# cornellius-gp/linear_operator

Hardware: AMD Instinct MI355X
Metric: cg_member_matvecs_per_sec (higher is better)
Workload: dtype f32

## Files before the change

linear_operator_amd/csrc/lo_cg.hip:

```cpp
#include <algorithm>
#include <chrono>
#include <cstddef>
#include <cmath>
#include <atomic>
#include <cstdlib>
#include <cstring>
#include <new>

#include "lo_device.h"
#include "lo_internal.h"
#include "lo_cg_onchip.h"

namespace lo {

bool g_onchip_disabled = false;
int g_onchip_fused_timeouts = 0;
constexpr int kResidentBackoff0 = 16, kResidentBackoffMax = 4096;
static std::atomic<int> g_res_timeouts{0}, g_res_cooldown{0}, g_res_backoff{kResidentBackoff0}, g_res_rearms{0},
    g_res_inject{0};
bool resident_off() { return g_onchip_disabled || g_res_cooldown.load(std::memory_order_relaxed) > 0; }
void resident_tick() {
  int c = g_res_cooldown.load(std::memory_order_relaxed);
  while (c > 0 && !g_res_cooldown.compare_exchange_weak(c, c - 1, std::memory_order_relaxed)) {
  }
  if (c == 1) {
    g_res_rearms.fetch_add(1, std::memory_order_relaxed);
    fprintf(stderr, "liblo_amd: resident kernels re-armed after their cool-down\n");
  }
}
static void resident_untick() {
  int c = g_res_cooldown.load(std::memory_order_relaxed);
  while (c > 0 && !g_res_cooldown.compare_exchange_weak(c, c + 1, std::memory_order_relaxed)) {
  }
}
static bool resident_off_after_tick() { return g_onchip_disabled || g_res_cooldown.load(std::memory_order_relaxed) > 1; }
static void resident_return_injection() { g_res_inject.fetch_add(1, std::memory_order_relaxed); }
void resident_note_ok() { g_res_backoff.store(kResidentBackoff0, std::memory_order_relaxed); }
bool resident_take_injection() {
  int n = g_res_inject.load(std::memory_order_relaxed);
  while (n > 0 && !g_res_inject.compare_exchange_weak(n, n - 1, std::memory_order_relaxed)) {
// ... 80 lines not shown

constexpr int kLockstepMinCols = 4;

struct CgDev {
  int64_t B, N;
  int c, S, S_dot, S_rz;
  int n_tridiag, max_iter, n_tridiag_iter, T;
  float tol, eps, stop_after;
  int check_nan_first;
  float *x, *r, *p, *z, *Ap;
  float *pAp_part, *rr_part, *rz_part;
  float *rhs_norm, *rz, *alpha, *beta, *resid_norm, *prev_ar, *prev_beta;
  int *rhs_is_zero, *has_conv;
  float* t_mat;
  CgCtrl* ctrl;
  float* ctrl_part;
  unsigned long long* oc_gbuf;
  unsigned long long* oc_close;
  unsigned long long* ls_gbuf;
  unsigned long long* pf_gbuf;
  int* pf_ctr;
  unsigned long long* pf_gran;
  unsigned long long* sc_gbuf;
  int* sc_ctr;
  unsigned long long* sc_gran;
  int* oc_err;
  float* oc_resid;
  int* oc_init_conv;
  float* oc_zero_q;
  float* oc_ones;
  float* oc_ab;
  int* oc_maxoff;
  long long* oc_dbg;
  double* rs_ws;
};

__global__ __launch_bounds__(kThreads) void k_cg_init_scal(CgDev d, const float* __restrict__ part) {
  const int64_t n = d.B * d.c;
  for (int64_t i = threadIdx.x; i < n; i += kThreads) {
    const int64_t b = i / d.c;
    const int col = (int)(i % d.c);
    float acc = 0.f;
    for (int s = 0; s < d.S; ++s) acc += part[(b * d.S + s) * d.c + col];
    float nrm = sqrtf(acc);
    const int zero = nrm < d.eps;
    d.rhs_is_zero[i] = zero;
    d.rhs_norm[i] = zero ? 1.0f : nrm;
  }
}

__global__ __launch_bounds__(kThreads) void k_cg_init_vec(CgDev d, const float* __restrict__ rhs,
                                                           const float* __restrict__ x0, int rows_per) {
  const int s = blockIdx.x, b = blockIdx.y;
  const int c = d.c, N = (int)d.N;
  const int nrs = kThreads / c;
  const int col = threadIdx.x % c, slot = threadIdx.x / c;
  if (slot >= nrs) return;
  const int r0 = s * rows_per, r1 = min(N, r0 + rows_per);
  const float nrm = d.rhs_norm[(size_t)b * c + col];
  const size_t base = (size_t)b * N * c + col;
  for (int row = r0 + slot; row < r1; row += nrs) {
    const size_t i = base + (size_t)row * c;
    d.r[i] = rhs[i] / nrm;
    d.x[i] = x0 ? x0[i] / nrm : 0.f;
  }
}
// ... 375 lines not shown
      cg_step_cols_worthwhile(B, N, c, pre != nullptr))
    out->streaming_precond = pre ? LO_STREAM_PRE_FUSED_COLS : LO_STREAM_NOPRE_FUSED_COLS;
  const bool opaque = (op->kind == LO_OP_CALLBACK) || pre_cb;
  out->poll_chunk = (opaque || global_rule) ? 1 : 4;
  const bool root_serial = serial.engine == LO_ENGINE_RESIDENT_ROOT;
  out->needs_q = (pre && !pre->Q && !(oc_ok && (ls_cols == c || root_serial))) ? 1 : 0;
  if (!oc_ok) return;
  out->resident = 1;
  out->resident_iterations = kfloor0 + 1;
  out->lockstep_cols = ls_cols;
  out->lockstep_group = ls_cols ? lockstep_group_size(N) : 0;
  if (ls_cols < c) {
    out->serial_engine = serial.engine;
    out->serial_group = serial.group;
  }
  out->lean = (!global_rule && !sw.keep_state && (ls_cols == c || root_serial)) ? 1 : 0;
  const bool rs_base = pre && pre->RS && pre_root && pre->rf_ld == RC && !global_rule && !sw.keep_state;
  if (rs_base && sh.rs_cols && (c >= 2 || prm->n_tridiag > 0) && !sw.no_rspace_cols) {
    out->rspace = 1;
    out->lean = 1;
  } else if (rs_base && out->lean && ls_cols == 0 && c == 1 && prm->n_tridiag == 0 && pre->E && root_serial &&
             rspace_eligible(RC, N, c) && !sw.no_rspace && !sw.no_wrec) {
    out->rspace = 2;
  }
}


static int oc_record_iters(const lo_cg_params* prm) {
  const int fmi0 = prm->floor_max_iter > 0 ? prm->floor_max_iter : prm->max_iter;
  int oc_iters = std::min(10, fmi0 - 1);
  if (prm->n_tridiag) oc_iters = std::max(oc_iters, std::min(prm->max_tridiag_iter, fmi0 - 1));
  return std::max(1, oc_iters + 1);
}

constexpr size_t kCgTail = 1024;
static int cg_layout(Arena& ar, const lo_op_desc* op, const lo_precond_desc* pre, bool pre_cb, const lo_cg_params* prm,
                     CgDev* d, MatvecPlan* pl, lo_matvec_cb mv_cb, void* mv_user, PrecondPlan* pp, hipStream_t st) {
  const int64_t B = op->B, N = op->N, c = prm->c;
  Split sp = choose_split(B, N, 256);
  const size_t nv = (size_t)B * N * c;
  const bool precond = pre != nullptr || pre_cb;
  CgDev& dd = *d;
  dd.B = B; dd.N = N; dd.c = (int)c; dd.S = sp.S;
  dd.ctrl = ar.take<CgCtrl>(1);
  dd.oc_gbuf = ar.take<unsigned long long>(std::max(onchip_gbuf_bytes(66), rspace_gbuf_bytes(std::max(66 * 8, 2 * onchip_num_workgroups()))) / sizeof(unsigned long long));
  dd.oc_close = ar.take<unsigned long long>((size_t)B + 2);
  dd.x = ar.take<float>(nv);
  dd.r = ar.take<float>(nv);
  dd.p = ar.take<float>(nv);
  dd.Ap = ar.take<float>(nv);
  dd.z = precond ? ar.take<float>(nv) : nullptr;
  dd.S_dot = matvec_S_dot(op, c, sp);
  dd.pAp_part = ar.take<float>((size_t)B * std::max(dd.S_dot, sp.S) * c);
  dd.rr_part = ar.take<float>((size_t)B * sp.S * c);
  dd.rz_part = precond ? ar.take<float>((size_t)B * sp.S * c) : dd.rr_part;
  dd.S_rz = sp.S;
  const size_t ns = (size_t)B * c;
  dd.rhs_norm = ar.take<float>(ns);
  dd.rz = ar.take<float>(ns);
  dd.alpha = ar.take<float>(ns);
  dd.beta = ar.take<float>(ns);
  dd.resid_norm = ar.take<float>(ns);
  dd.rhs_is_zero = ar.take<int>(ns);
  dd.has_conv = ar.take<int>(ns);
  const size_t nt = (size_t)B * std::max(1, (int)prm->n_tridiag);
  dd.prev_ar = ar.take<float>(nt);
  dd.prev_beta = ar.take<float>(nt);
  dd.ctrl_part = ar.take<float>(3 * 256);
  dd.oc_err = dd.ctrl ? &dd.ctrl->oc_err : nullptr;
  const int oc_iters = oc_record_iters(prm);
  const CgShape shp = cg_shape(op, pre, pre_cb, prm);
  const bool oc_shape = shp.oc_shape;
  const size_t oc_n = oc_shape ? (size_t)B * c : 1;
  dd.oc_resid = ar.take<float>(oc_n * oc_iters);
  dd.oc_init_conv = ar.take<int>(oc_n);
  dd.oc_ab = shp.has_ab ? ar.take<float>(2 * oc_n * oc_iters) : nullptr;
  dd.oc_maxoff = ar.take<int>((size_t)std::max(1, (int)prm->max_tridiag_iter) + 1);
  dd.oc_dbg = ar.take<long long>(16);
  dd.rs_ws = shp.rs_cols ? ar.take<double>(rspace_cols_ws_doubles(B, N, padded_rank(op->R), (int)c)) : nullptr;
  dd.ls_gbuf = shp.has_ls_gbuf
                   ? ar.take<unsigned long long>(lockstep_gbuf_bytes(32, 16) / sizeof(unsigned long long))
                   : nullptr;
  const bool pf_shape = shp.pf_shape;
  dd.pf_gbuf = pf_shape ? ar.take<unsigned long long>(precond_fused_gbuf_bytes() / sizeof(unsigned long long)) : nullptr;
  dd.pf_ctr = pf_shape ? ar.take<int>(2 * ((size_t)std::max(1, (int)prm->max_iter) + 1)) : nullptr;
  dd.pf_gran = pf_shape ? ar.take<unsigned long long>((size_t)B) : nullptr;
  dd.sc_gbuf = shp.sc_alloc ? ar.take<unsigned long long>(cg_step_cols_gbuf_bytes() / sizeof(unsigned long long)) : nullptr;
  dd.sc_ctr = shp.sc_alloc ? ar.take<int>(2 * ((size_t)std::max(1, (int)prm->max_iter) + 1)) : nullptr;
  dd.sc_gran = shp.sc_alloc ? ar.take<unsigned long long>(3 * (size_t)B) : nullptr;
  dd.oc_zero_q = nullptr;
  dd.oc_ones = nullptr;
  if (shp.has_zero_q) {
    dd.oc_zero_q = ar.take<float>((size_t)B * N * 4);
    dd.oc_ones = ar.take<float>((size_t)B);
  }
  int rc = pre ? precond_plan_init(pp, pre, B, N, c, sp, &ar, st) : LO_OK;
  const int rc_mv = matvec_plan_init(pl, op, mv_cb, mv_user, c, sp, &ar, st);
  if (!rc) rc = rc_mv;
  if (!rc && pl->S_dot != dd.S_dot) rc = LO_ERR_LAUNCH;
  return (rc || ar.ok) ? rc : LO_ERR_WORKSPACE;
}

struct CgDebug {
  bool ls = false, oc = false, sc = false;
  int member = 0;
  static CgDebug read(const CgEnv& env, int64_t B) {
    const bool ls = env.ls_debug && B >= 8, oc = !ls && env.oc_debug && B >= 8;
    return {ls, oc, env.sc_debug, oc ? env.oc_member : (ls ? env.ls_member : 0)};
  }
  int report_resident(const long long* dev) const {
    long long ts[12];
    if (ls) {
      LO_HIP_CHECK(hipMemcpy(ts, dev, 10 * sizeof(long long), hipMemcpyDeviceToHost));
      fprintf(stderr, "lockstep item (100 MHz ticks): load+H %lld init %lld iters %lld store %lld | direction %lld "
              "alpha+x+r %lld reduce-mfma %lld cross-wave %lld group-sum %lld\n",
              ts[1] - ts[0], ts[2] - ts[1], ts[3] - ts[2], ts[4] - ts[3], ts[5], ts[6], ts[7], ts[8], ts[9]);
    }
    if (oc) {
      LO_HIP_CHECK(hipMemcpy(ts, dev, 12 * sizeof(long long), hipMemcpyDeviceToHost));
      if (ts[8] || ts[9])
        fprintf(stderr, "  root-form kernel phases: updates %lld, w partials + all-reduce %lld, first-wave algebra %lld\n",
                ts[8], ts[9], ts[10]);
      fprintf(stderr, "onchip member0 (100 MHz ticks): load %lld init %lld iters %lld store %lld | wg-wait %lld publish %lld poll %lld\n",
              ts[1] - ts[0], ts[2] - ts[1], ts[3] - ts[2], ts[4] - ts[3], ts[5], ts[6], ts[7]);
    }
    return LO_OK;
  }
  int report_streaming(const long long* dev) const {
    if (!sc) return LO_OK;
    long long ts[8];
    LO_HIP_CHECK(hipMemcpy(ts, dev, sizeof(ts), hipMemcpyDeviceToHost));
    if (ts[5])
      fprintf(stderr, "cg_step_cols member 0, first workgroup (100 MHz ticks per launch): loads+alpha %.1f update+mfma %.1f "
              "all-reduce %.1f beta+control %.1f p %.1f\n", (double)ts[0] / ts[5], (double)ts[1] / ts[5], (double)ts[2] / ts[5],
              (double)ts[3] / ts[5], (double)ts[4] / ts[5]);
    return LO_OK;
  }
};

struct CgSolve {
  const lo_op_desc* op;
  const lo_precond_desc* pre;
  lo_matvec_cb precond_cb;
  void* precond_user;
  const lo_cg_params* prm;
  const float *rhs, *x0;
  float* x;
  hipStream_t st;
  int64_t B, N;
  int c;
  CgDev d;
  MatvecPlan pl;
  PrecondPlan pp = {};
  Split sp;
  int fmi, oc_nwg;
  bool precond, global_rule, oc_nopre;
  CgSwitches sw;
// ... 93 lines not shown
};

static int resident_close(CgSolve& s, const OnchipArgs& a, bool lean, bool dense, bool rs_cols_ran, unsigned close_ticket,
                          OcNext* next) {
  CgDev& d = s.d; const lo_cg_params* prm = s.prm; hipStream_t st = s.st; CgCtrl& h = s.h;
  const int ktri = prm->n_tridiag ? std::min(a.iters, (int)prm->max_tridiag_iter) : 0;
  const unsigned tri_grid = (unsigned)(((size_t)s.B * std::max(1, (int)prm->n_tridiag) + kThreads - 1) / kThreads);
  if (ktri) {
    LO_HIP_CHECK(hipMemsetAsync(d.oc_maxoff, 0, sizeof(int) * (prm->max_tridiag_iter + 1), st));
    hipLaunchKernelGGL(k_oc_maxoff, dim3(tri_grid), s.block, 0, st, d, d.oc_ab, ktri);
  }
  CgCtrl* mirror = static_cast<CgCtrl*>(pinned_status_block());
  const unsigned ticket = close_ticket ? close_ticket : next_ticket();
  if (!close_ticket)
    hipLaunchKernelGGL(k_cg_ctrl_onchip, dim3(1), s.block, 0, st, d, d.oc_resid, d.oc_init_conv, a.iters, ktri, mirror,
                       ticket);
  if (ktri) hipLaunchKernelGGL(k_oc_tridiag, dim3(tri_grid), s.block, 0, st, d, d.oc_ab, ktri);
  LO_LAUNCH_CHECK();
  if (mirror) {
    if (ktri) LO_HIP_CHECK(hipStreamSynchronize(st));
    else if (wait_ticket(reinterpret_cast<volatile unsigned*>(mirror) + 63, ticket, st)) return LO_ERR_LAUNCH;
    if (g_prof_host) tls_host_ticket = std::chrono::steady_clock::now();
    memcpy(&h, mirror, sizeof(CgCtrl));
  } else {
    LO_HIP_CHECK(hipMemcpyAsync(&h, d.ctrl, sizeof(CgCtrl), hipMemcpyDeviceToHost, st));
    LO_HIP_CHECK(hipStreamSynchronize(st));
  }
  int rc = LO_OK;
  if (h.oc_err == 0) {
    if (s.owned_launch) handoff_launch_confirm(s.owned_launch);
    rc = cg_global_check(s);
    if (rc) return rc;
  }
  rc = s.dbg.report_resident(d.oc_dbg);
  if (rc) return rc;
  if (h.oc_err == 0 && lean && h.rs_redo && tls_rspace_diag_ran && !dense) {
    *next = OcNext::kRedoDense;
  } else if (h.oc_err == 0 && lean && !h.stop) {
    lean_miss_note(s.op, prm, s.pre ? s.pre->generation : 0);
    if (s.pre && !s.pre->Q) return LO_ERR_UNSUPPORTED;
    *next = OcNext::kRedoState;
  } else if (h.oc_err == 0) {
    s.k_start = a.iters; s.x_written = true;
    resident_note_ok();
    lo_cg_plan& ex = s.exec;
    ex.resident = 1;
    if (rs_cols_ran) ex.lockstep_cols = 0, ex.serial_engine = LO_ENGINE_NONE;
    ex.lean = lean ? 1 : 0;
    ex.rspace = rs_cols_ran ? 1 : ((lean && tls_rspace_resident_ran) ? 2 : 0);
    ex.rspace_diag = (ex.rspace == 2 && tls_rspace_diag_ran) ? 1 : 0;
    *next = OcNext::kDone;
  } else {
    fprintf(stderr, "liblo_amd: operator-resident CG timed out, falling back to the streaming engine\n");
    onchip_note_timeout();
    if (s.ws_cleared) LO_HIP_CHECK(hipMemsetAsync(d.ctrl, 0, sizeof(CgCtrl), st));
    memset(&h, 0, sizeof(h));
    *next = OcNext::kStream;
  }
  return LO_OK;
}

static int resident_attempt(CgSolve& s, int attempt, bool lean, bool dense, OcNext* next) {
  CgDev& d = s.d; const lo_precond_desc* pre = s.pre; const lo_cg_params* prm = s.prm; lo_cg_plan& ex = s.exec;
  const int64_t B = s.B, N = s.N; const int c = s.c, RC = s.pl.lr.R4, ocR4 = s.oc_nopre ? 4 : s.pp.R4;
  hipStream_t st = s.st;
  *next = OcNext::kStream;
  OnchipArgs a;
  a.C = s.pl.lr.Apad; a.d = s.op->d; a.d_mode = s.op->diag_mode;
  if (s.oc_nopre) {
    if (ex.lockstep_cols < c && ex.serial_engine == LO_ENGINE_RESIDENT_GEN2) {
      LO_HIP_CHECK(hipMemsetAsync(d.oc_zero_q, 0, sizeof(float) * (size_t)B * N * 4, st));
      LO_HIP_CHECK(hipMemsetD32Async((hipDeviceptr_t)d.oc_ones, 0x3f800000, (size_t)B, st));
    }
    a.Q = d.oc_zero_q; a.dinv = d.oc_ones; a.dinv_mode = LO_DIAG_CONST;
  } else {
    a.Q = s.pp.Qp; a.dinv = pre->dinv; a.dinv_mode = pre->constant_diag ? LO_DIAG_CONST : LO_DIAG_FULL;
  }
  a.rhs = s.rhs; a.B = B; a.N = (int)N; a.c = c; a.ab_rec = prm->n_tridiag ? d.oc_ab : nullptr;
  a.col0 = 0; a.ncols = c; a.RK = s.pp.R4; a.RCg = RC;
  a.F = nullptr; a.EF = nullptr; a.E = nullptr; a.RS = nullptr; a.RSD = nullptr;
  a.close_gran = nullptr; a.close_count = nullptr; a.close_ctrl = nullptr; a.close_mirror = nullptr;
  a.close_ticket = 0; a.close_tol = 0.f; a.close_floor_ok = 0;
  a.close_epoch = 0x80000000u; a.tag_base = 0; a.handoff_owned = 0;
  a.iters = s.plan.first_stop_iteration + 1; a.eps = prm->eps; a.stop_after = prm->stop_updating_after;
  a.x = d.x; a.r = d.r; a.p = d.p; a.z = d.z;
  auto lean_state = [&](bool on) {
    a.x = on ? nullptr : d.x; a.r = on ? nullptr : d.r; a.p = on ? nullptr : d.p; a.z = on ? nullptr : d.z;
  };
  a.rhs_norm = d.rhs_norm; a.rz = d.rz; a.alpha = d.alpha; a.beta = d.beta; a.resid_norm = d.resid_norm;
  a.rhs_is_zero = d.rhs_is_zero; a.has_conv = d.has_conv;
  a.resid_rec = d.oc_resid; a.init_conv = d.oc_init_conv; a.err = d.oc_err;
  a.allow_l2_handoff = onchip_l2_handoff_allowed();
  a.prefetch = 1;
  a.dbg = nullptr; a.dbg_member = s.dbg.member;
  const bool injected = attempt == 0 && resident_take_injection();
  const bool inject = s.sw.oc_test_fallback || injected;
  s.owned_launch = 0;
  if (inject && s.ws_cleared) LO_HIP_CHECK(hipMemsetAsync(d.oc_err, 1, 1, st));
  if (s.dbg.oc || s.dbg.ls) LO_HIP_CHECK(hipMemsetAsync(d.oc_dbg, 0, 16 * sizeof(long long), st));
  int rc = LO_OK; int ls = ex.lockstep_cols;
  bool rs_cols_ran = false;
  unsigned close_ticket = 0;
  if (s.plan.rspace == 1 && lean && d.rs_ws) {
    a.xout = s.x;
    lean_state(true);
    a.F = pre->F; a.EF = pre->EF; a.E = pre->E; a.RS = pre->RS; a.RSD = pre->RSD;
    rc = rspace_cols_launch(RC, a, d.rs_ws, st);
    if (rc == LO_OK) {
      rs_cols_ran = true;
      ls = 0;
    } else if (rc != LO_ERR_UNSUPPORTED) {
      return rc;
    }
  }
  if (ls) {
    a.ncols = ls;
    a.xout = s.x;
    lean_state(lean);
    a.gbuf = d.ls_gbuf; a.next_member = d.oc_err + 2;
    a.dbg = s.dbg.ls ? d.oc_dbg : nullptr;
    LO_HIP_CHECK(hipMemsetAsync(d.ls_gbuf, 0, lockstep_gbuf_bytes(32, 16), st));
    a.GW = ex.lockstep_group;
    a.RW = (int)((N + a.GW - 1) / a.GW);
    rc = lockstep_launch(RC, pre != nullptr, a, std::min(s.oc_nwg, 256), st);
    if (rc == LO_ERR_UNSUPPORTED && a.GW == 16) {
      a.GW = ex.lockstep_group = 8;
      a.RW = (int)((N + 7) / 8);
      rc = lockstep_launch(RC, pre != nullptr, a, std::min(s.oc_nwg, 256), st);
    }
    if (rc == LO_ERR_UNSUPPORTED) {
      ex.lockstep_cols = ls = 0;
      ex.lockstep_group = 0;
// ... 595 lines not shown
```

linear_operator_amd/csrc/lo_cg_onchip.h:

```cpp
#pragma once
#include <stdint.h>

#include <hip/hip_runtime.h>

namespace lo {

struct CgCtrl;

struct OnchipArgs {
  const float* C;
  const float* Q;
  const float* d;
  const float* dinv;
  int d_mode, dinv_mode;
  const float* rhs;
  int c;
  int col0, ncols;
  int RK;
  int RCg;
  const float* F;
  const float* EF;
  const float* E;
  const double* RS;
  const double* RSD;
  float* ab_rec;
  int64_t B;
  int N, RW;
  int GW;
  int iters;
  float eps, stop_after;
  float *x, *r, *p, *z;
  float* xout;
  float *rhs_norm, *rz, *alpha, *beta, *resid_norm;
  int *rhs_is_zero, *has_conv;
  float* resid_rec;
  int* init_conv;
  unsigned long long* gbuf;
  int* err;
  int* next_member;
  int prefetch;
  int allow_l2_handoff;
  unsigned long long* close_gran;
  int* close_count;
  unsigned close_epoch;
  unsigned tag_base;
  int handoff_owned;
  struct CgCtrl* close_ctrl;
  struct CgCtrl* close_mirror;
  unsigned close_ticket;
  float close_tol;
  int close_floor_ok;
  long long* dbg;
  int dbg_member;
};

int onchip4_launch(int RC, int RK, const OnchipArgs& a, int nwg, hipStream_t st);
int onchip5_launch(int RC, const OnchipArgs& a, int nwg, hipStream_t st);
bool onchip5_eligible(int RC, int64_t N, int64_t c);
int rspace_launch(int RC, const OnchipArgs& a, int nwg, hipStream_t st);
int rspace3_launch(int RC, const OnchipArgs& a, int nwg, hipStream_t st);
int rspace3_launch_owned(int RC, const OnchipArgs& a, int nwg, bool inject, unsigned* launch_id, hipStream_t st);
void handoff_launch_confirm(unsigned launch_id);
bool rspace_eligible(int RC, int64_t N, int64_t c);
size_t rspace_gbuf_bytes(int nworkgroups);
extern thread_local bool tls_rspace_diag_ran;
extern thread_local bool tls_rspace_resident_ran;
int rspace_cols_launch(int RC, const OnchipArgs& a, double* ws, hipStream_t st);
bool rspace_cols_eligible(int RC, int64_t N, int64_t c);
size_t rspace_cols_ws_doubles(int64_t B, int64_t N, int RC, int c);
int lockstep_launch(int RC, bool pre, const OnchipArgs& a, int nwg, hipStream_t st);
bool lockstep_eligible(int RC, int RK, bool pre, int64_t N, int64_t ncols);
size_t lockstep_gbuf_bytes(int ngroups, int GW);
int lockstep_group_size(int64_t N);

}
```

linear_operator_amd/csrc/lo_rspace3.hip:

```cpp
#include <algorithm>
#include <atomic>
#include <mutex>
#include <type_traits>
#include <stdlib.h>

#include "lo_device.h"
#include "lo_internal.h"
#include "lo_cg_onchip.h"
#include "lo_group_reduce.h"
#include "lo_cg_close.h"
#include "lo_f64_lanes.h"

namespace lo {

namespace {

typedef float f32x4 __attribute__((ext_vector_type(4)));
typedef __attribute__((address_space(1))) const f32x4 g_cf4;
typedef __attribute__((address_space(1))) const float g_cf;
typedef __attribute__((address_space(1))) float g_f;
typedef __attribute__((address_space(1))) const char g_cc;
template <class T>
__device__ __forceinline__ T* opaque_uniform(T* p) {
  asm volatile("" : "+s"(p));
// ... 9 lines not shown
  long long member_off;
};
PeerOut g_peer_out = {{nullptr, nullptr, nullptr, nullptr, nullptr, nullptr, nullptr}, 0, 0};
std::mutex g_peer_mu;

__host__ __device__ constexpr int r3_np(int RC) { return 2 * RC + 6; }

__device__ __forceinline__ unsigned xor4_dpp_u(unsigned x) {
  const int a = __builtin_amdgcn_update_dpp(0, (int)x, 0x104, 0xf, 0x5, false);
  return (unsigned)__builtin_amdgcn_update_dpp(a, (int)x, 0x114, 0xf, 0xa, false);
}
__device__ __forceinline__ double halve4_d(double lo, double hi, int lane) {
  const bool up = (lane & 4) != 0;
  const double keep = up ? hi : lo;
  const double send = up ? lo : hi;
  return keep + mk_d(xor4_dpp_u(lo_w(send)), xor4_dpp_u(hi_w(send)));
}

template <int CH>
__device__ __forceinline__ double rows_reduce_d(double (&p)[CH], int lane) {
  if constexpr (CH == 8) {
#pragma unroll
    for (int m = 0; m < 4; ++m) p[m] = halve4_d(p[m], p[m + 4], lane);
    p[0] = halve_pair_d<2>(p[0], p[2], lane);
    p[1] = halve_pair_d<2>(p[1], p[3], lane);
    return halve_pair_d<1>(p[0], p[1], lane);
  } else if constexpr (CH == 4) {
    p[0] = halve_pair_d<2>(p[0], p[2], lane);
    p[1] = halve_pair_d<2>(p[1], p[3], lane);
    return halve_pair_d<1>(p[0], p[1], lane);
  } else {
    return halve_pair_d<1>(p[0], p[1], lane);
  }
}

template <int RC, int GW>
__global__ __launch_bounds__(R3_TPB, 2) void k_cg_rspace3(OnchipArgs a, PeerOut po) {
  constexpr int CH = RC / 4;
  constexpr int RPI = 64 / CH;
  constexpr int NI = 256 / RPI;
  constexpr int NP = r3_np(RC);
  constexpr int MLD = RC + 2;
  constexpr int NH = RC / 2;
  constexpr int NG = 2 * GW * NP;
  __shared__ __attribute__((aligned(16))) float bst[4][256];
  __shared__ __attribute__((aligned(16))) float dst[4][256];
  __shared__ __attribute__((aligned(16))) double mat_s[3 * RC * MLD];
  __shared__ __attribute__((aligned(16))) double red[4][NP];
  __shared__ __attribute__((aligned(16))) double res[NP];
  __shared__ __attribute__((aligned(16))) double gv[4][32];
  __shared__ unsigned polw[GW > 1 ? NG : 2];
  const GroupPlace gp = group_place(GW, (int)gridDim.x / 8);
  if (!gp.active) return;
  const int grp = gp.grp, wig = gp.wig, ngroups = gp.ngroups;
  const int t = threadIdx.x, lane = t & 63, wave = t >> 6;
  const int wave_u = __builtin_amdgcn_readfirstlane(wave);
  unsigned long long* const gbase = a.gbuf + (size_t)grp * 2 * NG;
  unsigned tag = a.tag_base;
  bool same_xcd = false;
  const unsigned xcc = xcc_id();
  bool first = true;
  const int row0 = wig * R3_ROWS + 256 * wave_u;
  const int row0c = max(0, min(row0, a.N - 256));
  const bool di_full = a.dinv_mode == LO_DIAG_FULL;
  float* const bw = bst[wave_u];
  float* const dw = dst[wave_u];
  constexpr int NPF = 8;
  f32x4 pre[NPF];
  constexpr int NXT = NI - NPF;
  f32x4 nxt[NXT > 0 ? NXT : 1];
  auto request = [&](int64_t bm, int tl_, int i_lo, auto cnt, f32x4* dst) {
    const int ln_ = tl_ & 63, k_ = ln_ & (CH - 1), g_ = ln_ / CH;
    const unsigned loff = (unsigned)((g_ * RC + 4 * k_) * sizeof(float));
    g_cc* Cw = (g_cc*)(a.C + ((size_t)bm * a.N + row0c) * RC);
#pragma unroll
    for (int q = 0; q < decltype(cnt)::value / 8; ++q) {
      g_cc* bq = opaque_uniform(Cw + (i_lo + 8 * q + 4) * 1024);
#pragma unroll
      for (int i = 0; i < 8; ++i) dst[8 * q + i] = *(g_cf4*)(bq + loff + (i - 4) * 1024);
    }
  };
  int64_t b = grp;
  {
    int tl0 = t;
    asm volatile("" : "+v"(tl0));
    if (b < a.B) {
      request(b, tl0, 0, std::integral_constant<int, NPF>{}, pre);
      request(b, tl0, NPF, std::integral_constant<int, NXT>{}, nxt);
    } else {
#pragma unroll
      for (int i = 0; i < NPF; ++i) pre[i] = (f32x4){0.f, 0.f, 0.f, 0.f};
    }
  }
  while (b < a.B) {
    const bool stamp = a.dbg && b == a.dbg_member && wig == 0 && t == 0;
    if (stamp) a.dbg[0] = wall_clock64();
    int drawn = 0;
    if (wig == 0 && t == 0) drawn = atomicAdd(a.next_member, 1);
    int tl = t;
    asm volatile("" : "+v"(tl));
    const int ln = tl & 63, k = ln & (CH - 1), g = ln / CH;
    f32x4 Cr[NI];
#pragma unroll
    for (int i = 0; i < NPF; ++i) Cr[i] = pre[i];
#pragma unroll
    for (int i = 0; i < NXT; ++i) Cr[NPF + i] = nxt[i];
    float bq4[4], dq4[4];
    {
      g_cf* bb_ = opaque_uniform((g_cf*)(a.rhs + (size_t)b * a.N + row0c));
      g_cf* dd_ = opaque_uniform((g_cf*)(di_full ? a.dinv + (size_t)b * a.N + row0c : a.dinv + b));
      const int lo_e = row0 - row0c, hi_e = max(0, min(256, a.N - row0c));
      const int dstride = di_full ? 1 : 0;
#pragma unroll
      for (int m = 0; m < 4; ++m) {
        const int e = ln + 64 * m;
        const bool own = e >= lo_e && e < hi_e;
        bq4[m] = own ? bb_[e] : 0.f;
        dq4[m] = own ? dd_[e * dstride] : 0.f;
      }
    }
    constexpr int NM = (3 * RC * RC / 2 + R3_TPB - 1) / R3_TPB;
    f32x4 mv[NM];
    {
      typedef __attribute__((address_space(1))) const f32x4 g_m4;
      const g_m4* src = (const g_m4*)(a.RSD + (size_t)b * 6 * RC * RC);
#pragma unroll
      for (int u = 0; u < NM; ++u) {
        const int e = min(tl + R3_TPB * u, 3 * RC * RC / 2 - 1);
        const int ms = e / (RC * RC / 2);
        const int mg = ms == 0 ? 0 : ms + 1;
        mv[u] = src[(size_t)mg * (RC * RC / 2) + (e - ms * (RC * RC / 2))];
      }
    }
    const double lam_mine = a.RSD[((size_t)b * 6 + 5) * RC * RC + min(ln & 31, RC - 1)];
#pragma unroll
    for (int m = 0; m < 4; ++m) {
      bw[ln + 64 * m] = bq4[m];
      dw[ln + 64 * m] = dq4[m];
    }
#pragma unroll
    for (int u = 0; u < NM; ++u) {
      const int e = tl + R3_TPB * u;
      if (e < 3 * RC * RC / 2) {
        const int mi = e / (RC / 2), jj = e % (RC / 2);
        *reinterpret_cast<f32x4*>(&mat_s[mi * MLD + 2 * jj]) = mv[u];
      }
    }
    __builtin_amdgcn_wave_barrier();
    if (stamp) a.dbg[1] = wall_clock64();

    {
      double aw[4] = {0.0, 0.0, 0.0, 0.0}, au[4] = {0.0, 0.0, 0.0, 0.0};
#pragma unroll
      for (int i0 = 0; i0 < NI; i0 += 4) {
#pragma unroll
        for (int i = i0; i < i0 + 4; ++i) {
          const int r = RPI * i + g;
          const double bb = (double)bw[r];
          const double bd = bb * (double)dw[r];
          const double c0 = (double)Cr[i].x, c1 = (double)Cr[i].y, c2 = (double)Cr[i].z, c3 = (double)Cr[i].w;
          aw[0] = fma(c0, bd, aw[0]); au[0] = fma(c0, bb, au[0]);
          aw[1] = fma(c1, bd, aw[1]); au[1] = fma(c1, bb, au[1]);
          aw[2] = fma(c2, bd, aw[2]); au[2] = fma(c2, bb, au[2]);
          aw[3] = fma(c3, bd, aw[3]); au[3] = fma(c3, bb, au[3]);
        }
        __builtin_amdgcn_sched_barrier(0);
      }
      double s_acc = 0.0, a_acc = 0.0, d2_acc = 0.0;
#pragma unroll
      for (int j = 0; j < 4; ++j) {
        const int rw = 64 * j + RPI * k + g;
        const double bb = (double)bw[rw], di = (double)dw[rw];
        s_acc = fma(bb, bb * di, s_acc);
        a_acc = fma(bb, bb, a_acc);
        d2_acc = fma(di, di, d2_acc);
      }
      double h0 = halve_pair_d<32>(aw[0], au[0], ln), h1 = halve_pair_d<32>(aw[1], au[1], ln);
      double h2 = halve_pair_d<32>(aw[2], au[2], ln), h3 = halve_pair_d<32>(aw[3], au[3], ln);
      h0 = halve_pair_d<16>(h0, h2, ln);
      h1 = halve_pair_d<16>(h1, h3, ln);
      double mine = halve_pair_d<8>(h0, h1, ln);
      if constexpr (CH <= 4) mine = bfly_add_d<4>(mine);
// ... 47 lines not shown
              x[q] = granule_load(slot + min(idx, NG - 1));
              ok = ok && (granule_tag(x[q]) == tag);
            }
            if (ok) break;
            if (poll_give_up(spin, a.err)) {
              lost = true;
              break;
            }
            __builtin_amdgcn_s_sleep(1);
          }
#pragma unroll
          for (int q = 0; q < CKQ; ++q) {
            const int idx = tt + R3_TPB * (q0 + q);
            if (idx < NG) polw[idx] = granule_bits(x[q]);
          }
        }
        __syncthreads();
        if (tt < NP) {
          double tot = 0.0;
#pragma unroll
          for (int w = 0; w < GW; ++w) tot += mk_d(polw[(w * NP + tt) * 2], polw[(w * NP + tt) * 2 + 1]);
          res[tt] = tot;
        }
      }
      __syncthreads();
    }
    if (GW > 1 && first) {
      unsigned xc = xcc;
      asm volatile("" : "+s"(xc));
      same_xcd = same_xcd_verdict(res[2 * RC + 4], res[2 * RC + 5], GW, xc, a.allow_l2_handoff);
    }
    first = false;
    if (stamp) a.dbg[2] = wall_clock64();
    const int64_t b_next = (int64_t)res[2 * RC + 2];
    {
      int tp = t;
      asm volatile("" : "+v"(tp));
      if (b_next < a.B) {
        request(b_next, tp, 0, std::integral_constant<int, NPF>{}, pre);
      } else {
#pragma unroll
        for (int i = 0; i < NPF; ++i) pre[i] = (f32x4){0.f, 0.f, 0.f, 0.f};
      }
    }
    if (a.prefetch & 1) __builtin_amdgcn_s_setprio(3);

    const int j = lane & 31, hf = lane >> 5;
    const bool live = j < RC;
    const int jr = live ? j : RC - 1;
    double yj = 0.0, xi = 0.0;
    float nrm;
    {
      double a0 = res[2 * RC + 1], s = res[2 * RC];
      const double d2 = res[2 * RC + 3];
      nrm = sqrtf((float)a0);
      const bool rhs_zero = nrm < a.eps;
      if (rhs_zero) nrm = 1.0f;
      const double inv = 1.0 / (double)nrm;
      const double w0 = live ? res[jr] * inv : 0.0, u0 = live ? res[RC + jr] * inv : 0.0;
      s *= inv * inv;
      a0 *= inv * inv;
      float sa = a.stop_after;
      asm volatile("" : "+s"(sa));
      const double sure_rz = 2.0 * (double)sa * (double)sa * sqrt(d2);
      auto own_row_dot = [&](const double* mrow, const double* vec) {
        double a0_ = 0.0, a1_ = 0.0;
#pragma unroll
        for (int q = 0; q < NH; q += 2) {
          const double2 xa = *reinterpret_cast<const double2*>(mrow + q);
          const double2 xx = *reinterpret_cast<const double2*>(vec + q);
          a0_ = fma(xa.x, xx.x, a0_);
          a1_ = fma(xa.y, xx.y, a1_);
        }
        double lo_, up_;
        halves_d(a0_ + a1_, lo_, up_);
        return lo_ + up_;
      };
      double* myv = gv[wave];
      if (hf == 0) myv[j] = w0;
      __builtin_amdgcn_wave_barrier();
      const double* row0m = mat_s + (size_t)jr * MLD + hf * NH;
      double c0 = own_row_dot(row0m, myv + hf * NH);
      double e0 = own_row_dot(row0m + (size_t)1 * RC * MLD, myv + hf * NH);
      const double* nrow = row0m + (size_t)2 * RC * MLD;
      const double* tucol = mat_s + (size_t)(1 * RC + hf * NH) * MLD + jr;
      c0 = live ? c0 : 0.0;
      e0 = live ? e0 : 0.0;
      double tau2 = s - lanes32_sum_d(c0 * e0);
      tau2 = tau2 > 0.0 ? tau2 : 0.0;
      const bool delicate = !rhs_zero && tau2 < 1e-2 * s;
      const double lam = live ? lam_mine : 1.0;
      long long ts_a = 0, ts_b = 0;
      if (stamp) ts_a = wall_clock64();
      double cj = c0, qj = 0.0, etaj = 0.0;
      double cp = 1.0, qp = 0.0, etap = 0.0;
      double rz = 0.0, pApE = 0.0, alpha = 0.0, beta = 0.0;
      float rn = 0.f, last_alpha = 0.f;
      bool conv = false;
      unsigned close_flags = 0u;
      const size_t bc = (size_t)b;
      const bool rec = wig == 0 && lane == 0;
      const int last_owner = (a.iters - 1) & 3;
      for (int kk = -1; kk < a.iters; ++kk) {
        if (kk >= 0) {
          last_alpha = (float)alpha;
          etaj = fma(alpha, qj, etaj);
          etap = fma(alpha, qp, etap);
          cj = fma(-alpha * lam, qj, cj);
          cp = fma(-alpha, qp, cp);
        }
        const double lc = lam * cj;
        const bool lo_h = hf == 0;
        const float inv_rz = __builtin_amdgcn_rcpf((float)rz);
        const double red2 = row16_sum_d(halve_pair_d<16>(lo_h ? cj * cj : lc * qj, lo_h ? lc * cj : 0.0, lane));
        const auto pick = [&](double v, int ln_) {
          return mk_d((unsigned)__builtin_amdgcn_readlane((int)lo_w(v), ln_),
                      (unsigned)__builtin_amdgcn_readlane((int)hi_w(v), ln_));
        };
        const double cc = pick(red2, 0), clc = pick(red2, 16), clq = pick(red2, 32);
        const double rzn = fma(cp * cp, tau2, cc);
        const bool sure = rzn > sure_rz;
        const bool rec_first = kk == 0 && a.close_gran == nullptr && wave == 0;
        const bool rec_last = kk == a.iters - 1 && wave == last_owner;
        const bool own = rec_first || rec_last || !sure;
        float rnn = 0.f;
        if (kk < 0) {
          const float s1f = (float)a0;
          rnn = __builtin_amdgcn_sqrtf(s1f < 0.f ? 0.f : s1f);
        } else if (own) {
          const double dl = fma(-cp, c0, cj);
          __builtin_amdgcn_wave_barrier();
          if (hf == 0) myv[j] = dl;
          __builtin_amdgcn_wave_barrier();
          double gj_;
          {
            double a0_ = 0.0, a1_ = 0.0;
#pragma unroll
            for (int q = 0; q < NH; q += 2) {
              const double2 dd = *reinterpret_cast<const double2*>(myv + hf * NH + q);
              a0_ = fma(tucol[(size_t)q * MLD], dd.x, a0_);
              a1_ = fma(tucol[(size_t)(q + 1) * MLD], dd.y, a1_);
            }
            double lo_, up_;
            halves_d(a0_ + a1_, lo_, up_);
            gj_ = live ? lo_ + up_ : 0.0;
          }
          __builtin_amdgcn_wave_barrier();
          if (hf == 0) myv[j] = gj_;
          __builtin_amdgcn_wave_barrier();
          const double nd = own_row_dot(nrow, myv + hf * NH);
          const double r2 = row16_sum_d(halve_pair_d<16>(gj_ * nd, gj_ * u0, lane));
          const double dnd = pick(r2, 0), dm = pick(r2, 16);
          const double s1 = fma(cp, fma(cp, a0, 2.0 * dm), dnd);
          const float s1f = (float)s1;
          rnn = __builtin_amdgcn_sqrtf(s1f < 0.f ? 0.f : s1f);
        }
        if (kk >= 0) {
          beta = ((float)rz < a.eps) ? 0.0 : (double)((float)rzn * inv_rz);
          if (rhs_zero) rnn = 0.f;
          rn = rnn;
          if (rec && (rec_first || rec_last)) a.resid_rec[(size_t)kk * a.B + bc] = rn;
        } else {
          beta = 0.0;
          rn = rnn;
          if (wig == 0 && t == 0) a.init_conv[bc] = (rn < a.stop_after) ? 1 : 0;
          close_flags = ((rn < a.stop_after) ? 1u : 0u) | (delicate ? 4u : 0u);
          if (delicate && rec && wave == 0) atomicOr(a.err + 4, 1);
        }
        if (kk == 0 && (rnn != rnn || rzn != rzn)) close_flags |= 2u;
        conv = (own || rhs_zero) ? (rn < a.stop_after) : false;
        rz = rzn;
        pApE = fma(beta, fma(beta, pApE, 2.0 * clq), clc);
        qj = fma(beta, qj, cj);
        qp = fma(beta, qp, cp);
        const double pAp = fma(qp * qp, tau2, pApE);
        alpha = ((float)pAp < a.eps) ? 0.0 : (double)((float)rz * __builtin_amdgcn_rcpf((float)pAp));
        if (conv) alpha = 0.0;
      }
      if (stamp) ts_b = wall_clock64();
      if (rec && wave == last_owner) {
        a.rhs_norm[bc] = nrm;
        a.rhs_is_zero[bc] = rhs_zero ? 1 : 0;
        a.rz[bc] = (float)rz;
        a.alpha[bc] = last_alpha;
        a.beta[bc] = (float)beta;
        a.resid_norm[bc] = rn;
        a.has_conv[bc] = conv ? 1 : 0;
        if (a.close_gran) {
          granule_store(a.close_gran + b, granule_pack(a.close_epoch | close_flags, rn), false);
        }
      }
      __builtin_amdgcn_wave_barrier();
      if (hf == 0) myv[j] = fma(-etap, e0, etaj);
      __builtin_amdgcn_wave_barrier();
      xi = etap;
      {
        const double* col = mat_s + (size_t)(hf * NH) * MLD + jr;
        double a0_ = 0.0, a1_ = 0.0;
#pragma unroll
        for (int q = 0; q < NH; q += 2) {
          const double2 ee = *reinterpret_cast<const double2*>(myv + hf * NH + q);
          a0_ = fma(col[(size_t)q * MLD], ee.x, a0_);
          a1_ = fma(col[(size_t)(q + 1) * MLD], ee.y, a1_);
        }
        double lo_, up_;
        halves_d(a0_ + a1_, lo_, up_);
        yj = lo_ + up_;
      }
      yj = live ? yj : 0.0;
      if (stamp) {
        a.dbg[5] = ts_a - a.dbg[2];
        a.dbg[6] = ts_b - ts_a;
        a.dbg[7] = wall_clock64() - ts_b;
      }
      __builtin_amdgcn_wave_barrier();
      if (hf == 0) myv[j] = yj * (double)nrm;
      __builtin_amdgcn_wave_barrier();
    }
    if (!(a.prefetch & 2)) __builtin_amdgcn_s_setprio(0);
    if (stamp) a.dbg[3] = wall_clock64();
    {
      int l2 = lane;
      asm volatile("" : "+v"(l2));
      const int k2 = l2 & (CH - 1), g2 = l2 / CH;
      const double* myv = gv[wave];
      const double2 ya = *reinterpret_cast<const double2*>(&myv[4 * k2]);
      const double2 yb = *reinterpret_cast<const double2*>(&myv[4 * k2 + 2]);
      g_f* const xb = opaque_uniform((g_f*)(a.xout + (size_t)b * a.N + row0c));
      const bool more = b_next < a.B;
      g_cc* const Cn = (g_cc*)(a.C + ((size_t)(more ? b_next : b) * a.N + row0c) * RC);
      const unsigned loffn = (unsigned)((g2 * RC + 4 * k2) * sizeof(float));
#pragma unroll
      for (int js = 0; js < 4; ++js) {
        constexpr int J0 = NPF / CH;
        const int jj = (js + J0) & 3;
        double p[CH];
#pragma unroll
        for (int m = 0; m < CH; ++m) {
          const f32x4 c4 = Cr[CH * jj + m];
          p[m] = fma((double)c4.w, yb.y, fma((double)c4.z, yb.x, fma((double)c4.y, ya.y, (double)c4.x * ya.x)));
        }
        const double xv = rows_reduce_d<CH>(p, l2);
        const int rw = 64 * jj + RPI * k2 + g2;
        const int row = row0c + rw;
        const double acc = fma(xi, (double)bw[rw], xv);
        if (row >= row0 && row < a.N) {
          const float xval = (float)(acc * (double)dw[rw]);
          xb[rw] = xval;
          for (int pp = 0; pp < po.n; ++pp)
            ((g_f*)po.buf[pp])[((size_t)(b + po.member_off)) * a.N + row] = xval;
        }
        if (CH * jj >= NPF) {
          g_cc* bqn = opaque_uniform(Cn + (CH * jj + 4) * 1024);
#pragma unroll
          for (int m = 0; m < CH; ++m)
            nxt[CH * jj - NPF + m] = more ? *(g_cf4*)(bqn + loffn + (m - 4) * 1024) : (f32x4){0.f, 0.f, 0.f, 0.f};
        }
      }
      __builtin_amdgcn_wave_barrier();
    }
    __builtin_amdgcn_s_setprio(0);
    if (stamp) a.dbg[4] = wall_clock64();
    __syncthreads();
    b = b_next;
  }
  if (a.close_gran && wig == 0) cg_close_solve(a, ngroups, t);
}

int rspace3_prio() {
  static const int prio = [] {
    const char* e = getenv("LO_RS_PRIO");
    return e ? atoi(e) : 3;
  }();
  return prio;
}

constexpr size_t HO_MAX_WGS = 2 * 320;
constexpr size_t HO_GRAN_PER_WG = 432;
constexpr size_t HO_MAX_MEMBERS = 65536;
constexpr size_t HO_HEAD_BYTES = 256;
constexpr unsigned HO_TAG_LIMIT = 0xfff00000u;
constexpr unsigned HO_EPOCH_LIMIT = 0x1ffffff0u;
struct HandoffBlock {
  char* buf = nullptr;
  size_t bytes = 0;
  bool failed = false;
  unsigned next_tag = 1, next_epoch = 1;
  unsigned last_launch = 0;
  std::atomic<unsigned> confirmed{0};
  bool force_clear = false;
  unsigned clears = 0, launches = 0;
};
HandoffBlock g_handoff[16];
std::atomic<unsigned> g_handoff_ids{0};

HandoffBlock* handoff_block() {
  int dev = 0;
// ... 148 lines not shown
```

Measured before the change: 36.68 million.

## Defer last-iteration residual record to overlap with next member's load

The final CG iteration's residual walk and record stores are peeled out of the per-member loop and run later. For small group widths they run after the next member's data load begins, using a double-buffered shared-memory matrix image; otherwise they run after the x write-back. This takes the serial tail off the critical path between members, at the cost of doubled LDS for the matrix image, extra shared staging state, and a per-member debug timeline buffer.

```diff
diff --git a/linear_operator_amd/csrc/lo_cg.hip b/linear_operator_amd/csrc/lo_cg.hip
--- a/linear_operator_amd/csrc/lo_cg.hip
+++ b/linear_operator_amd/csrc/lo_cg.hip
@@ -6,6 +6,7 @@
 #include <cstdlib>
 #include <cstring>
 #include <new>
+#include <vector>
 
 #include "lo_device.h"
 #include "lo_internal.h"
@@ -152,6 +153,7 @@
   float* oc_ab;
   int* oc_maxoff;
   long long* oc_dbg;
+  int64_t oc_dbg_members;
   double* rs_ws;
 };
 
@@ -593,6 +595,8 @@
   if (prm->n_tridiag) oc_iters = std::max(oc_iters, std::min(prm->max_tridiag_iter, fmi0 - 1));
   return std::max(1, oc_iters + 1);
 }
+
+static size_t oc_dbg_words(int64_t members) { return kOcDbgHead + (size_t)kOcDbgTimeline * (size_t)members; }
 
 constexpr size_t kCgTail = 1024;
 static int cg_layout(Arena& ar, const lo_op_desc* op, const lo_precond_desc* pre, bool pre_cb, const lo_cg_params* prm,
@@ -637,7 +641,8 @@
   dd.oc_init_conv = ar.take<int>(oc_n);
   dd.oc_ab = shp.has_ab ? ar.take<float>(2 * oc_n * oc_iters) : nullptr;
   dd.oc_maxoff = ar.take<int>((size_t)std::max(1, (int)prm->max_tridiag_iter) + 1);
-  dd.oc_dbg = ar.take<long long>(16);
+  dd.oc_dbg_members = (oc_shape && c == 1) ? B : 0;
+  dd.oc_dbg = ar.take<long long>(oc_dbg_words(dd.oc_dbg_members));
   dd.rs_ws = shp.rs_cols ? ar.take<double>(rspace_cols_ws_doubles(B, N, padded_rank(op->R), (int)c)) : nullptr;
   dd.ls_gbuf = shp.has_ls_gbuf
                    ? ar.take<unsigned long long>(lockstep_gbuf_bytes(32, 16) / sizeof(unsigned long long))
@@ -669,7 +674,7 @@
     const bool ls = env.ls_debug && B >= 8, oc = !ls && env.oc_debug && B >= 8;
     return {ls, oc, env.sc_debug, oc ? env.oc_member : (ls ? env.ls_member : 0)};
   }
-  int report_resident(const long long* dev) const {
+  int report_resident(const long long* dev, int64_t members) const {
     long long ts[12];
     if (ls) {
       LO_HIP_CHECK(hipMemcpy(ts, dev, 10 * sizeof(long long), hipMemcpyDeviceToHost));
@@ -684,6 +689,16 @@
                 ts[8], ts[9], ts[10]);
       fprintf(stderr, "onchip member0 (100 MHz ticks): load %lld init %lld iters %lld store %lld | wg-wait %lld publish %lld poll %lld\n",
               ts[1] - ts[0], ts[2] - ts[1], ts[3] - ts[2], ts[4] - ts[3], ts[5], ts[6], ts[7]);
+      if (members > 0) {
+        std::vector<long long> tl((size_t)kOcDbgTimeline * (size_t)members);
+        LO_HIP_CHECK(hipMemcpy(tl.data(), dev + kOcDbgHead, tl.size() * sizeof(long long), hipMemcpyDeviceToHost));
+        for (int64_t m = 0; m < members; ++m) {
+          const long long* w = tl.data() + (size_t)kOcDbgTimeline * (size_t)m;
+          if (w[0])
+            fprintf(stderr, "rs3-timeline member %lld group %lld stamps %lld %lld %lld %lld %lld\n", (long long)m, w[0] - 1, w[1],
+                    w[2], w[3], w[4], w[5]);
+        }
+      }
     }
     return LO_OK;
   }
@@ -843,7 +858,7 @@
     rc = cg_global_check(s);
     if (rc) return rc;
   }
-  rc = s.dbg.report_resident(d.oc_dbg);
+  rc = s.dbg.report_resident(d.oc_dbg, d.oc_dbg_members);
   if (rc) return rc;
   if (h.oc_err == 0 && lean && h.rs_redo && tls_rspace_diag_ran && !dense) {
     *next = OcNext::kRedoDense;
@@ -903,12 +918,12 @@
   a.resid_rec = d.oc_resid; a.init_conv = d.oc_init_conv; a.err = d.oc_err;
   a.allow_l2_handoff = onchip_l2_handoff_allowed();
   a.prefetch = 1;
-  a.dbg = nullptr; a.dbg_member = s.dbg.member;
+  a.dbg = nullptr; a.dbg_member = s.dbg.member; a.dbg_timeline = d.oc_dbg_members;
   const bool injected = attempt == 0 && resident_take_injection();
   const bool inject = s.sw.oc_test_fallback || injected;
   s.owned_launch = 0;
   if (inject && s.ws_cleared) LO_HIP_CHECK(hipMemsetAsync(d.oc_err, 1, 1, st));
-  if (s.dbg.oc || s.dbg.ls) LO_HIP_CHECK(hipMemsetAsync(d.oc_dbg, 0, 16 * sizeof(long long), st));
+  if (s.dbg.oc || s.dbg.ls) LO_HIP_CHECK(hipMemsetAsync(d.oc_dbg, 0, oc_dbg_words(d.oc_dbg_members) * sizeof(long long), st));
   int rc = LO_OK; int ls = ex.lockstep_cols;
   bool rs_cols_ran = false;
   unsigned close_ticket = 0;
diff --git a/linear_operator_amd/csrc/lo_cg_onchip.h b/linear_operator_amd/csrc/lo_cg_onchip.h
--- a/linear_operator_amd/csrc/lo_cg_onchip.h
+++ b/linear_operator_amd/csrc/lo_cg_onchip.h
@@ -52,7 +52,10 @@
   int close_floor_ok;
   long long* dbg;
   int dbg_member;
+  int64_t dbg_timeline;
 };
+constexpr int kOcDbgHead = 16;
+constexpr int kOcDbgTimeline = 6;
 
 int onchip4_launch(int RC, int RK, const OnchipArgs& a, int nwg, hipStream_t st);
 int onchip5_launch(int RC, const OnchipArgs& a, int nwg, hipStream_t st);
diff --git a/linear_operator_amd/csrc/lo_rspace3.hip b/linear_operator_amd/csrc/lo_rspace3.hip
--- a/linear_operator_amd/csrc/lo_rspace3.hip
+++ b/linear_operator_amd/csrc/lo_rspace3.hip
@@ -65,6 +65,69 @@
   } else {
     return halve_pair_d<1>(p[0], p[1], lane);
   }
+}
+
+__device__ __forceinline__ double pick_d(double v, int ln) {
+  return mk_d((unsigned)__builtin_amdgcn_readlane((int)lo_w(v), ln), (unsigned)__builtin_amdgcn_readlane((int)hi_w(v), ln));
+}
+
+template <int NH>
+__device__ __forceinline__ double half_row_dot_d(const double* mrow, const double* vec) {
+  double a0_ = 0.0, a1_ = 0.0;
+#pragma unroll
+  for (int q = 0; q < NH; q += 2) {
+    const double2 xa = *reinterpret_cast<const double2*>(mrow + q);
+    const double2 xx = *reinterpret_cast<const double2*>(vec + q);
+    a0_ = fma(xa.x, xx.x, a0_);
+    a1_ = fma(xa.y, xx.y, a1_);
+  }
+  double lo_, up_;
+  halves_d(a0_ + a1_, lo_, up_);
+  return lo_ + up_;
+}
+
+template <int RC>
+__device__ __forceinline__ float resid_walk_d(double* vec, const double* tucol, const double* nrow, double cj, double cp,
+                                              double c0, double u0, double a0, bool live, int j, int hf, int lane) {
+  constexpr int MLD = RC + 2, NH = RC / 2;
+  const double dl = fma(-cp, c0, cj);
+  __builtin_amdgcn_wave_barrier();
+  if (hf == 0) vec[j] = dl;
+  __builtin_amdgcn_wave_barrier();
+  double gj_;
+  {
+    double a0_ = 0.0, a1_ = 0.0;
+#pragma unroll
+    for (int q = 0; q < NH; q += 2) {
+      const double2 dd = *reinterpret_cast<const double2*>(vec + hf * NH + q);
+      a0_ = fma(tucol[(size_t)q * MLD], dd.x, a0_);
+      a1_ = fma(tucol[(size_t)(q + 1) * MLD], dd.y, a1_);
+    }
+    double lo_, up_;
+    halves_d(a0_ + a1_, lo_, up_);
+    gj_ = live ? lo_ + up_ : 0.0;
+  }
+  __builtin_amdgcn_wave_barrier();
+  if (hf == 0) vec[j] = gj_;
+  __builtin_amdgcn_wave_barrier();
+  const double nd = half_row_dot_d<NH>(nrow, vec + hf * NH);
+  const double r2 = row16_sum_d(halve_pair_d<16>(gj_ * nd, gj_ * u0, lane));
+  const double dnd = pick_d(r2, 0), dm = pick_d(r2, 16);
+  const double s1 = fma(cp, fma(cp, a0, 2.0 * dm), dnd);
+  const float s1f = (float)s1;
+  return __builtin_amdgcn_sqrtf(s1f < 0.f ? 0.f : s1f);
+}
+
+__device__ __forceinline__ void store_records(const OnchipArgs& a, int64_t b, float nrm, bool rhs_zero, float rz, float alpha,
+                                              float beta, float rn, bool conv, unsigned close_flags) {
+  a.rhs_norm[b] = nrm;
+  a.rhs_is_zero[b] = rhs_zero ? 1 : 0;
+  a.rz[b] = rz;
+  a.alpha[b] = alpha;
+  a.beta[b] = beta;
+  a.resid_norm[b] = rn;
+  a.has_conv[b] = conv ? 1 : 0;
+  if (a.close_gran) granule_store(a.close_gran + b, granule_pack(a.close_epoch | close_flags, rn), false);
 }
 
 template <int RC, int GW>
@@ -78,10 +141,18 @@
   constexpr int NG = 2 * GW * NP;
   __shared__ __attribute__((aligned(16))) float bst[4][256];
   __shared__ __attribute__((aligned(16))) float dst[4][256];
-  __shared__ __attribute__((aligned(16))) double mat_s[3 * RC * MLD];
+  constexpr bool TAIL_LATE = GW <= 8;
+  constexpr int MAT_N = 3 * RC * MLD;
+  __shared__ __attribute__((aligned(16))) double mat_im[(TAIL_LATE ? 2 : 1) * MAT_N];
   __shared__ __attribute__((aligned(16))) double red[4][NP];
   __shared__ __attribute__((aligned(16))) double res[NP];
   __shared__ __attribute__((aligned(16))) double gv[4][32];
+  __shared__ __attribute__((aligned(16))) double tl_g[32];
+  __shared__ __attribute__((aligned(16))) double tl_v[3][64];
+  __shared__ __attribute__((aligned(16))) double tl_sc[4];
+  __shared__ float tl_f[2];
+  __shared__ unsigned tl_u[2];
+  __shared__ long long tl_b[1];
   __shared__ unsigned polw[GW > 1 ? NG : 2];
   const GroupPlace gp = group_place(GW, (int)gridDim.x / 8);
   if (!gp.active) return;
@@ -125,9 +196,52 @@
       for (int i = 0; i < NPF; ++i) pre[i] = (f32x4){0.f, 0.f, 0.f, 0.f};
     }
   }
+  const auto record_tail = [&](const double* mat_s) {
+    int lt = lane;
+    asm volatile("" : "+v"(lt));
+    const int jt = lt & 31, hft = lt >> 5;
+    const bool live_t = jt < RC;
+    const int jrt = live_t ? jt : RC - 1;
+    __builtin_amdgcn_wave_barrier();
+    const double cj = tl_v[0][lt], c0 = tl_v[1][lt], u0 = tl_v[2][lt];
+    const double cp = tl_sc[0], a0 = tl_sc[1], tau2 = tl_sc[2], rz = tl_sc[3];
+    const float nrm_t = tl_f[0], last_alpha = tl_f[1];
+    const bool rhs_zero = tl_u[0] != 0u;
+    unsigned close_flags = tl_u[1];
+    const int64_t bt = tl_b[0];
+    const int kk = a.iters - 1;
+    const float inv_rz = __builtin_amdgcn_rcpf((float)rz);
+    const double red2 = row16_sum_d(halve_pair_d<16>(hft == 0 ? cj * cj : 0.0, 0.0, lt));
+    const double cc = pick_d(red2, 0);
+    const double rzn = fma(cp * cp, tau2, cc);
+    const double* nrow = mat_s + (size_t)(2 * RC + jrt) * MLD + hft * NH;
+    const double* tucol = mat_s + (size_t)(1 * RC + hft * NH) * MLD + jrt;
+    float rnn = resid_walk_d<RC>(tl_g, tucol, nrow, cj, cp, c0, u0, a0, live_t, jt, hft, lt);
+    const double beta = ((float)rz < a.eps) ? 0.0 : (double)((float)rzn * inv_rz);
+    if (rhs_zero) rnn = 0.f;
+    const float rn = rnn;
+    if (kk == 0 && (rnn != rnn || rzn != rzn)) close_flags |= 2u;
+    const bool conv = rn < a.stop_after;
+    if (lt == 0) {
+      a.resid_rec[(size_t)kk * a.B + (size_t)bt] = rn;
+      store_records(a, bt, nrm_t, rhs_zero, (float)rzn, last_alpha, (float)beta, rn, conv, close_flags);
+    }
+  };
+  bool tail_pending = false;
+  int img = 0;
   while (b < a.B) {
     const bool stamp = a.dbg && b == a.dbg_member && wig == 0 && t == 0;
     if (stamp) a.dbg[0] = wall_clock64();
+    const bool tline = a.dbg && b < a.dbg_timeline && wig == 0 && t == 0;
+    const auto tl_word = [&](int i) { return a.dbg + kOcDbgHead + kOcDbgTimeline * (long long)__builtin_amdgcn_readfirstlane((int)b) + i; };
+    const auto tl_stamp = [&](int i) { *tl_word(i) = wall_clock64(); };
+    if (tline) {
+      int gq = grp + 1;
+      asm volatile("" : "+s"(gq));
+      *tl_word(0) = gq;
+      tl_stamp(1);
+    }
+    double* const mat_s = mat_im + (TAIL_LATE ? img * MAT_N : 0);
     int drawn = 0;
     if (wig == 0 && t == 0) drawn = atomicAdd(a.next_member, 1);
     int tl = t;
@@ -166,6 +280,10 @@
       }
     }
     const double lam_mine = a.RSD[((size_t)b * 6 + 5) * RC * RC + min(ln & 31, RC - 1)];
+    if constexpr (TAIL_LATE) {
+      if (tail_pending) record_tail(mat_im + (img ^ 1) * MAT_N);
+      tail_pending = false;
+    }
 #pragma unroll
     for (int m = 0; m < 4; ++m) {
       bw[ln + 64 * m] = bq4[m];
@@ -181,6 +299,7 @@
     }
     __builtin_amdgcn_wave_barrier();
     if (stamp) a.dbg[1] = wall_clock64();
+    if (tline) tl_stamp(2);
 
     {
       double aw[4] = {0.0, 0.0, 0.0, 0.0}, au[4] = {0.0, 0.0, 0.0, 0.0};
@@ -294,6 +413,7 @@
     }
     first = false;
     if (stamp) a.dbg[2] = wall_clock64();
+    if (tline) tl_stamp(3);
     const int64_t b_next = (int64_t)res[2 * RC + 2];
     {
       int tp = t;
@@ -325,19 +445,7 @@
       float sa = a.stop_after;
       asm volatile("" : "+s"(sa));
       const double sure_rz = 2.0 * (double)sa * (double)sa * sqrt(d2);
-      auto own_row_dot = [&](const double* mrow, const double* vec) {
-        double a0_ = 0.0, a1_ = 0.0;
-#pragma unroll
-        for (int q = 0; q < NH; q += 2) {
-          const double2 xa = *reinterpret_cast<const double2*>(mrow + q);
-          const double2 xx = *reinterpret_cast<const double2*>(vec + q);
-          a0_ = fma(xa.x, xx.x, a0_);
-          a1_ = fma(xa.y, xx.y, a1_);
-        }
-        double lo_, up_;
-        halves_d(a0_ + a1_, lo_, up_);
-        return lo_ + up_;
-      };
+      const auto own_row_dot = [](const double* mrow, const double* vec) { return half_row_dot_d<NH>(mrow, vec); };
       double* myv = gv[wave];
       if (hf == 0) myv[j] = w0;
       __builtin_amdgcn_wave_barrier();
@@ -363,7 +471,8 @@
       const size_t bc = (size_t)b;
       const bool rec = wig == 0 && lane == 0;
       const int last_owner = (a.iters - 1) & 3;
-      for (int kk = -1; kk < a.iters; ++kk) {
+      const int full_end = a.iters > 0 ? a.iters - 1 : 0;
+      for (int kk = -1; kk < full_end; ++kk) {
         if (kk >= 0) {
           last_alpha = (float)alpha;
           etaj = fma(alpha, qj, etaj);
@@ -375,53 +484,23 @@
         const bool lo_h = hf == 0;
         const float inv_rz = __builtin_amdgcn_rcpf((float)rz);
         const double red2 = row16_sum_d(halve_pair_d<16>(lo_h ? cj * cj : lc * qj, lo_h ? lc * cj : 0.0, lane));
-        const auto pick = [&](double v, int ln_) {
-          return mk_d((unsigned)__builtin_amdgcn_readlane((int)lo_w(v), ln_),
-                      (unsigned)__builtin_amdgcn_readlane((int)hi_w(v), ln_));
-        };
-        const double cc = pick(red2, 0), clc = pick(red2, 16), clq = pick(red2, 32);
+        const double cc = pick_d(red2, 0), clc = pick_d(red2, 16), clq = pick_d(red2, 32);
         const double rzn = fma(cp * cp, tau2, cc);
         const bool sure = rzn > sure_rz;
         const bool rec_first = kk == 0 && a.close_gran == nullptr && wave == 0;
-        const bool rec_last = kk == a.iters - 1 && wave == last_owner;
-        const bool own = rec_first || rec_last || !sure;
+        const bool own = rec_first || !sure;
         float rnn = 0.f;
         if (kk < 0) {
           const float s1f = (float)a0;
           rnn = __builtin_amdgcn_sqrtf(s1f < 0.f ? 0.f : s1f);
         } else if (own) {
-          const double dl = fma(-cp, c0, cj);
-          __builtin_amdgcn_wave_barrier();
-          if (hf == 0) myv[j] = dl;
-          __builtin_amdgcn_wave_barrier();
-          double gj_;
-          {
-            double a0_ = 0.0, a1_ = 0.0;
-#pragma unroll
-            for (int q = 0; q < NH; q += 2) {
-              const double2 dd = *reinterpret_cast<const double2*>(myv + hf * NH + q);
-              a0_ = fma(tucol[(size_t)q * MLD], dd.x, a0_);
-              a1_ = fma(tucol[(size_t)(q + 1) * MLD], dd.y, a1_);
-            }
-            double lo_, up_;
-            halves_d(a0_ + a1_, lo_, up_);
-            gj_ = live ? lo_ + up_ : 0.0;
-          }
-          __builtin_amdgcn_wave_barrier();
-          if (hf == 0) myv[j] = gj_;
-          __builtin_amdgcn_wave_barrier();
-          const double nd = own_row_dot(nrow, myv + hf * NH);
-          const double r2 = row16_sum_d(halve_pair_d<16>(gj_ * nd, gj_ * u0, lane));
-          const double dnd = pick(r2, 0), dm = pick(r2, 16);
-          const double s1 = fma(cp, fma(cp, a0, 2.0 * dm), dnd);
-          const float s1f = (float)s1;
-          rnn = __builtin_amdgcn_sqrtf(s1f < 0.f ? 0.f : s1f);
+          rnn = resid_walk_d<RC>(myv, tucol, nrow, cj, cp, c0, u0, a0, live, j, hf, lane);
         }
         if (kk >= 0) {
           beta = ((float)rz < a.eps) ? 0.0 : (double)((float)rzn * inv_rz);
           if (rhs_zero) rnn = 0.f;
           rn = rnn;
-          if (rec && (rec_first || rec_last)) a.resid_rec[(size_t)kk * a.B + bc] = rn;
+          if (rec && rec_first) a.resid_rec[(size_t)kk * a.B + bc] = rn;
         } else {
           beta = 0.0;
           rn = rnn;
@@ -439,19 +518,36 @@
         alpha = ((float)pAp < a.eps) ? 0.0 : (double)((float)rz * __builtin_amdgcn_rcpf((float)pAp));
         if (conv) alpha = 0.0;
       }
+      const bool tail_wave = wig == 0 && wave_u == last_owner;
+      if (a.iters > 0) {
+        last_alpha = (float)alpha;
+        etaj = fma(alpha, qj, etaj);
+        etap = fma(alpha, qp, etap);
+        cj = fma(-alpha * lam, qj, cj);
+        cp = fma(-alpha, qp, cp);
+        tail_pending = tail_wave;
+        if (tail_wave) {
+          int ls = lane;
+          asm volatile("" : "+v"(ls));
+          tl_v[0][ls] = cj;
+          tl_v[1][ls] = c0;
+          tl_v[2][ls] = u0;
+          if (ls == 0) {
+            tl_sc[0] = cp;
+            tl_sc[1] = a0;
+            tl_sc[2] = tau2;
+            tl_sc[3] = rz;
+            tl_f[0] = nrm;
+            tl_f[1] = last_alpha;
+            tl_u[0] = rhs_zero ? 1u : 0u;
+            tl_u[1] = close_flags;
+            tl_b[0] = b;
+          }
+        }
+      } else if (rec && tail_wave) {
+        store_records(a, b, nrm, rhs_zero, (float)rz, last_alpha, (float)beta, rn, conv, close_flags);
+      }
       if (stamp) ts_b = wall_clock64();
-      if (rec && wave == last_owner) {
-        a.rhs_norm[bc] = nrm;
-        a.rhs_is_zero[bc] = rhs_zero ? 1 : 0;
-        a.rz[bc] = (float)rz;
-        a.alpha[bc] = last_alpha;
-        a.beta[bc] = (float)beta;
-        a.resid_norm[bc] = rn;
-        a.has_conv[bc] = conv ? 1 : 0;
-        if (a.close_gran) {
-          granule_store(a.close_gran + b, granule_pack(a.close_epoch | close_flags, rn), false);
-        }
-      }
       __builtin_amdgcn_wave_barrier();
       if (hf == 0) myv[j] = fma(-etap, e0, etaj);
       __builtin_amdgcn_wave_barrier();
@@ -481,6 +577,7 @@
     }
     if (!(a.prefetch & 2)) __builtin_amdgcn_s_setprio(0);
     if (stamp) a.dbg[3] = wall_clock64();
+    if (tline) tl_stamp(4);
     {
       int l2 = lane;
       asm volatile("" : "+v"(l2));
@@ -523,8 +620,17 @@
     }
     __builtin_amdgcn_s_setprio(0);
     if (stamp) a.dbg[4] = wall_clock64();
+    if (tline) tl_stamp(5);
+    if constexpr (!TAIL_LATE) {
+      if (tail_pending) record_tail(mat_s);
+      tail_pending = false;
+    }
     __syncthreads();
     b = b_next;
+    img ^= 1;
+  }
+  if constexpr (TAIL_LATE) {
+    if (tail_pending) record_tail(mat_im + (img ^ 1) * MAT_N);
   }
   if (a.close_gran && wig == 0) cg_close_solve(a, ngroups, t);
 }
```

New measurement: 37.24 million, median of 3. 1.02x the previous value.
